# matwilso/generative_models

Measured on AMD Instinct MI355X. Metric: ddpm_train_images_per_sec, higher is better.
Workload: dtype fp16_fwd+bf16_bwd; 1 GPU; DDPM train step, 3x32x32, SimpleUnet C=128, 2048 images per GPU, T=1000 (BASELINE.json configs[2]); key=cfg2, global_batch=2048, parallelism=dp1

## Files before the change

generative_models_amd/csrc/conv1x1_stream.hip:

```cpp
#include <type_traits>

#include "gmk_common.h"

namespace {

constexpr int kRow = 272;

template <typename T>
__global__ __launch_bounds__(256) void conv1x1_pair_stream_kernel(const T* __restrict__ src, const T* __restrict__ w, T* __restrict__ out_a,
                                                                 T* __restrict__ out_b, unsigned npix, unsigned ntiles, unsigned src_bytes) {
    fp16_saturating_stores<T>();
    typedef typename Frag16<T>::type frag_t;
    typedef __attribute__((ext_vector_type(4))) unsigned int u32x4s;
    constexpr unsigned kBadOff = 0xFFFFFF00u;
    __shared__ __attribute__((aligned(16))) char wl[256 * kRow];
    __shared__ __attribute__((aligned(16))) char tile[128 * kRow];
    __shared__ __attribute__((aligned(16))) char trans[4 * 32 * kRow];
    const int tid = threadIdx.x, lane = tid & 63, wave = tid >> 6;
    const int r = lane & 31, h = lane >> 5;
    const __amdgpu_buffer_rsrc_t rss = __builtin_amdgcn_make_buffer_rsrc(const_cast<T*>(src), 0, (int)src_bytes, 0x00020000);
    const __amdgpu_buffer_rsrc_t rsa = __builtin_amdgcn_make_buffer_rsrc(out_a, 0, (int)src_bytes, 0x00020000);
    const __amdgpu_buffer_rsrc_t rsb = __builtin_amdgcn_make_buffer_rsrc(out_b, 0, (int)src_bytes, 0x00020000);
#pragma unroll
    for (int i = 0; i < 16; ++i) {
// ... 145 lines not shown
                s16x4 hi = __builtin_amdgcn_ds_read_tr16_b64_v4i16((GMK_LDS s16x4*)(Yb + (pxl + 4) * 256 + wa));
                const s16x8 t = {lo[0], lo[1], lo[2], lo[3], hi[0], hi[1], hi[2], hi[3]};
                a[i] = __builtin_bit_cast(bf16x8, t);
                lo = __builtin_amdgcn_ds_read_tr16_b64_v4i16((GMK_LDS s16x4*)(Xb + pxl * 256 + wb));
                hi = __builtin_amdgcn_ds_read_tr16_b64_v4i16((GMK_LDS s16x4*)(Xb + (pxl + 4) * 256 + wb));
                const s16x8 u = {lo[0], lo[1], lo[2], lo[3], hi[0], hi[1], hi[2], hi[3]};
                b[i] = __builtin_bit_cast(bf16x8, u);
            }
#pragma unroll
            for (int i = 0; i < 2; ++i)
#pragma unroll
                for (int j = 0; j < 2; ++j) acc[i][j] = __builtin_amdgcn_mfma_f32_32x32x16_bf16(a[i], b[j], acc[i][j], 0, 0, 0);
        }
        if (ks + 1 < nk) write_step(PAR ^ 1, ry[PAR ^ 1], rx0[PAR ^ 1], rx1[PAR ^ 1]);
        __syncthreads();
    };
    for (int ks = 0; ks < nk; ks += 2) {
        k_step(ks, std::integral_constant<int, 0>{});
        if (ks + 1 < nk) k_step(ks + 1, std::integral_constant<int, 1>{});
    }
    float* out = slab + (int64_t)blockIdx.x * (128 * 256) + cib * 128;
#pragma unroll
    for (int i = 0; i < 2; ++i)
#pragma unroll
        for (int j = 0; j < 2; ++j)
#pragma unroll
            for (int e = 0; e < 16; ++e) {
                const int co = wm * 64 + i * 32 + (e & 3) + 8 * (e >> 2) + 4 * h;
                const int ci = wn * 64 + j * 32 + r;
                out[co * 256 + ci] = acc[i][j][e];
            }
}

}

int gmk_conv1x1_pair_stream_try(const void* src, int64_t npix, const void* w_rows256, void* out_a, void* out_b, int dtype, hipStream_t stream) {
    if (!gmk_is16(dtype) || gmk_kernel_choice(3, "GMK_DEV_VARIANT") == 46) return 0;
    const int64_t bytes = npix * 256;
    if (bytes >= 0xFFFFFF00ll) return 0;
    const int64_t ntiles = (npix + 127) / 128;
    const int ncu = gmk_cu_limit();
    if (ntiles < 2 * ncu) return 0;
    const unsigned grid = (unsigned)ncu;
    if (dtype == GMK_BF16)
        conv1x1_pair_stream_kernel<bf16_t><<<grid, 256, 0, stream>>>((const bf16_t*)src, (const bf16_t*)w_rows256, (bf16_t*)out_a, (bf16_t*)out_b,
                                                                    (unsigned)npix, (unsigned)ntiles, (unsigned)bytes);
    else
        conv1x1_pair_stream_kernel<f16_t><<<grid, 256, 0, stream>>>((const f16_t*)src, (const f16_t*)w_rows256, (f16_t*)out_a, (f16_t*)out_b,
                                                                   (unsigned)npix, (unsigned)ntiles, (unsigned)bytes);
    return 1;
}

int gmk_conv1x1_wgrad_stream_try(const void* dy, int dy_cstride, const void* src0, const void* src1, int64_t npix, float* slab, int64_t slab_bytes,
                                 bool x_f16, hipStream_t stream) {
    if (gmk_kernel_choice(3, "GMK_DEV_VARIANT") == 47) return 0;
    const int ncu = gmk_cu_limit();
    if (npix < (int64_t)ncu * 64 * 8 || npix >= (1ll << 31) - 64) return 0;
    if (slab_bytes < (int64_t)ncu * 128 * 256 * 4) return 0;
    int64_t chunk = (npix + ncu - 1) / ncu;
    chunk = (chunk + 63) / 64 * 64;
    const int ns = (int)((npix + chunk - 1) / chunk);
    if (x_f16)
        conv1x1_wgrad_stream_kernel<f16_t><<<ns, 512, 0, stream>>>((const bf16_t*)dy, dy_cstride, (const f16_t*)src0, (const f16_t*)src1, slab, (int)npix, (int)chunk);
    else
        conv1x1_wgrad_stream_kernel<bf16_t><<<ns, 512, 0, stream>>>((const bf16_t*)dy, dy_cstride, (const bf16_t*)src0, (const bf16_t*)src1, slab, (int)npix, (int)chunk);
    return ns;
}
```

generative_models_amd/csrc/conv_igemm.hip:

```cpp
#include <stdlib.h>

#include <type_traits>

#include "gmk_common.h"

namespace {

constexpr int kBM = 128, kBN = 128;

struct GatherParams {
    int hs, ws;
    int ho, wo;
    int ksize, pad;
    int mul, shift, mask, lim_h, lim_w;
    signed char ty[9], tx[9];
    unsigned char tapw[9];
    int ntaps;
    int oscale, ooy, oox, out_w, out_hw;
};

__host__ bool make_gather(int mode, int ksize, int hs, int ws, int ho, int wo, GatherParams* g) {
    g->hs = hs; g->ws = ws; g->ho = ho; g->wo = wo;
    g->ksize = ksize; g->pad = ksize == 3 ? 1 : 0;
    g->mul = 1; g->shift = 0; g->mask = 0; g->lim_h = hs; g->lim_w = ws;
// ... 1053 lines not shown
        dim3 grid((p.M + kBM - 1) / kBM, cout / kBN);
        if (dtype == GMK_BF16) conv_igemm_kernel<bf16_t><<<grid, 256, 0, gmk_stream(stream)>>>(p);
        else if (dtype == GMK_F16) conv_igemm_kernel<f16_t><<<grid, 256, 0, gmk_stream(stream)>>>(p);
        else if (fp32_split()) conv_igemm_kernel<float, true><<<grid, 256, 0, gmk_stream(stream)>>>(p);
        else conv_igemm_kernel<float><<<grid, 256, 0, gmk_stream(stream)>>>(p);
    }
    return gmk_check_launch("gmk_conv_igemm");
}

extern "C" int gmk_conv_igemm(const void* src0, const void* src1, int c0, int c1, int B, int hs, int ws, int ho, int wo,
                              int ksize, int mode, const void* w, int w_rows, int n0, int cout, const float* bias,
                              const float* emb, int emb_stride, const void* residual, void* out, int out_cstride,
                              float* gn_stats, int64_t gn_stats_bytes, const float* gn_scale, const float* gn_shift, int gn_stride,
                              int dtype, void* stream) {
    return conv_igemm_impl(src0, src1, c0, c1, B, hs, ws, ho, wo, ksize, mode, w, w_rows, n0, cout, bias, emb, emb_stride, residual,
                           out, nullptr, out_cstride, gn_stats, gn_stats_bytes, gn_scale, gn_shift, gn_stride, dtype, stream);
}

extern "C" int gmk_conv1x1_pair(const void* src, int c, int B, int H, int W, const void* w, int w_rows, int n0, void* out_a,
                                void* out_b, int dtype, void* stream) {
    GMK_REQUIRE(src && w && out_a && out_b, "gmk_conv1x1_pair: null pointer");
    GMK_REQUIRE(n0 >= 0 && n0 + 256 <= w_rows, "gmk_conv1x1_pair: rows n0 .. n0 + 255 outside the %d packed rows", w_rows);
    if (c == 128 && B > 0 && H > 0 && W > 0) {
        const size_t es = 2;
        if (gmk_conv1x1_pair_stream_try(src, (int64_t)B * H * W, (const char*)w + (size_t)n0 * 128 * es, out_a, out_b, dtype, gmk_stream(stream))) {
            gmk_note_kernel(14);
            return gmk_check_launch("gmk_conv1x1_pair(stream)");
        }
    }
    return conv_igemm_impl(src, nullptr, c, 0, B, H, W, H, W, 1, GMK_CONV_NORMAL, w, w_rows, n0, 128, nullptr, nullptr, 0, nullptr,
                           out_a, out_b, 128, nullptr, 0, nullptr, nullptr, 0, dtype, stream);
}

extern "C" int gmk_conv_gn_fusable(int B, int H, int W, int c0, int c1, int cout) {
    const int force = gmk_kernel_choice(0, "GMK_CONV_KERNEL");
    if (force != 0 && force != 3) return 0;
    return gmk_halo_geometry(B, H, W, c0, c1, cout, cout, cout, 1, 0, 1, nullptr);
}

extern "C" int gmk_conv_wgrad(const void* dy, int dy_cstride, const void* src0, const void* src1, int c0, int c1, int B,
                              int hs, int ws, int ho, int wo, int ksize, int mode, float* dw, int cout, void* workspace,
                              int64_t workspace_bytes, int dtype, int x_dtype, void* stream) {
    GMK_REQUIRE(dy && src0 && dw && workspace, "gmk_conv_wgrad: null pointer");
    GMK_REQUIRE(dtype == GMK_BF16 || dtype == GMK_F32, "gmk_conv_wgrad: bad dtype %d", dtype);
    GMK_REQUIRE(x_dtype == dtype || (dtype == GMK_BF16 && x_dtype == GMK_F16),
                "gmk_conv_wgrad: activations of type %d with gradients of type %d (same type, or fp16 activations with bf16 gradients)", x_dtype, dtype);
    const bool xf16 = x_dtype == GMK_F16;
    GMK_REQUIRE(ksize == 1 || ksize == 3, "gmk_conv_wgrad: ksize %d", ksize);
    GMK_REQUIRE(c0 > 0 && c0 % 128 == 0 && c1 >= 0 && c1 % 128 == 0 && (c1 == 0 || src1),
                "gmk_conv_wgrad: source channels must be multiples of 128 (c0=%d c1=%d)", c0, c1);
    GMK_REQUIRE(cout > 0 && cout % 128 == 0 && dy_cstride >= cout, "gmk_conv_wgrad: bad cout=%d", cout);
    GMK_REQUIRE(B > 0 && (int64_t)B * ho * wo < (1ll << 31) - 256 && (int64_t)B * hs * ws < (1ll << 31),
                "gmk_conv_wgrad: problem too large for 32-bit pixel indices");
    GMK_REQUIRE(mode != GMK_CONV_TRANSPOSED2, "gmk_conv_wgrad: no weight gradient for the transposed gather");
    WgradParams p;
    GMK_REQUIRE(make_gather(mode, ksize, hs, ws, ho, wo, &p.g), "gmk_conv_wgrad: mode %d inconsistent with %dx%d -> %dx%d",
                mode, hs, ws, ho, wo);
    const int taps = ksize * ksize;
    const int wforce = gmk_kernel_choice(1, "GMK_WGRAD_KERNEL");
    const bool s2 = mode == GMK_CONV_STRIDE2 && hs == 2 * ho && ws == 2 * wo;
    if (wforce != 1 && dtype == GMK_BF16 && (mode == GMK_CONV_NORMAL || mode == GMK_CONV_UPSAMPLE2 || s2) && ksize == 3) {
        const int ns2 = gmk_conv_wgrad_slots_try(dy, dy_cstride, src0, src1, c0, c1, B, ho, wo, cout, (float*)workspace,
                                                 workspace_bytes, wforce, mode == GMK_CONV_UPSAMPLE2, xf16, gmk_stream(stream), s2);
        if (ns2 > 0) {
            int rc2 = gmk_check_launch("gmk_conv_wgrad(slots)");
            if (rc2) return rc2;
// ... 35 lines not shown
```

generative_models_amd/csrc/gmk_common.h:

```cpp
#pragma once
#include <hip/hip_runtime.h>
#include <stdint.h>

#include "../../include/gmk.h"

typedef __bf16 bf16_t;
typedef __attribute__((ext_vector_type(8))) __bf16 bf16x8;
typedef __attribute__((ext_vector_type(4))) __bf16 bf16x4;
typedef _Float16 f16_t;
typedef __attribute__((ext_vector_type(8))) _Float16 f16x8;
typedef __attribute__((ext_vector_type(4))) _Float16 f16x4;
typedef __attribute__((ext_vector_type(2))) _Float16 f16x2;
typedef __attribute__((ext_vector_type(2))) __bf16 bf16x2;
typedef __attribute__((ext_vector_type(4))) short s16x4;
typedef __attribute__((ext_vector_type(4))) float f32x4;
typedef __attribute__((ext_vector_type(16))) float f32x16;

#define GMK_LDS __attribute__((address_space(3)))

void gmk_set_error(const char* fmt, ...);
int gmk_check_launch(const char* what);
int gmk_kernel_choice(int which, const char* env);
int gmk_conv1x1_pair_stream_try(const void* src, int64_t npix, const void* w_rows256, void* out_a, void* out_b, int dtype, hipStream_t stream);
int gmk_conv1x1_wgrad_stream_try(const void* dy, int dy_cstride, const void* src0, const void* src1, int64_t npix, float* slab, int64_t slab_bytes,
                                 bool x_f16, hipStream_t stream);
int gmk_conv_subpixel_takes(int B, int H, int W, int cin, int cout, int w_rows, int ntaps, int out_cstride, int dtype);
bool fp32_split(void);
int gmk_cu_limit(void);
void gmk_note_kernel(int id);

#define GMK_REQUIRE(cond, ...)                 \
    do {                                       \
        if (!(cond)) {                         \
            gmk_set_error(__VA_ARGS__);        \
            return GMK_ERR_ARG;                \
        }                                      \
    } while (0)

int gmk_conv3x3_halo_try(const void* src0, const void* src1, int c0, int c1, int B, int H, int W, const void* w, int w_rows,
                         int n0, int cout, const float* bias, const float* emb, int emb_stride, const void* residual,
                         void* out, int out_cstride, int min_tiles, int upsample, float* stats, int64_t stats_bytes,
                         const float* gn_scale, const float* gn_shift, int gn_stride, int dtype, hipStream_t stream);

struct HaloGeometry { int R, TP, slots; int64_t rows_total, M, ntiles, nb0, nb1, nbw, nbo; };
int gmk_halo_geometry(int B, int H, int W, int c0, int c1, int w_rows, int cout, int out_cstride, int min_tiles, int upsample,
                      int fused_gn, HaloGeometry* g);

int gmk_wgrad_slots_nsplit(int cout, int ktot);
int gmk_conv_wgrad_slots_try(const void* dy, int dy_cstride, const void* src0, const void* src1, int c0, int c1, int B, int H,
                             int W, int cout, float* slab, int64_t slab_bytes, int forced, int upsample, bool x_f16,
                             hipStream_t stream, int stride2 = 0);


static inline hipStream_t gmk_stream(void* s) { return reinterpret_cast<hipStream_t>(s); }
static inline int gmk_esize(int dtype) { return dtype == GMK_F32 ? 4 : 2; }
static inline bool gmk_is16(int dtype) { return dtype == GMK_BF16 || dtype == GMK_F16; }

template <typename T> struct Vec8;
// ... 145 lines not shown
```

generative_models_amd/diffusion/simple_unet.py:

```python
import math
import os
from collections import OrderedDict

import torch
from torch import nn

from .. import ops

MAX_TIMESTEPS = 256


def _res_names(prefix, cin, cout, emb):
    out = [
        (f"{prefix}.in_layers.0.weight", (cin,)), (f"{prefix}.in_layers.0.bias", (cin,)),
        (f"{prefix}.in_layers.2.weight", (cout, cin, 3, 3)), (f"{prefix}.in_layers.2.bias", (cout,)),
        (f"{prefix}.emb_layers.1.weight", (cout, emb)), (f"{prefix}.emb_layers.1.bias", (cout,)),
        (f"{prefix}.out_layers.0.weight", (cout,)), (f"{prefix}.out_layers.0.bias", (cout,)),
        (f"{prefix}.out_layers.3.weight", (cout, cout, 3, 3)), (f"{prefix}.out_layers.3.bias", (cout,)),
    ]
    if cin != cout:
        out += [(f"{prefix}.skip_connection.weight", (cout, cin, 1, 1)), (f"{prefix}.skip_connection.bias", (cout,))]
    return out


# ... 538 lines not shown
                ops.set_cu_limit(part[0] - part[1])
        for t in tensors:
            t.record_stream(side)

    def _emb_ready(self):
        pend = getattr(self, "_emb_pending", None)
        if pend is not None:
            self._emb_pending = None
            self._join_side()
            pend.record_stream(torch.cuda.current_stream())

    def _join_side(self):
        if self._side is not None:
            torch.cuda.current_stream().wait_stream(self._side)

    def _res_bwd(self, name, ctx, dout, dout_sum, demb_all, blk, extra_add=None, grads=True, defer_skip=False):
        P, G, C = self._pv, self._gv, self.channels
        srcs, a, stats1, h, a2, (mean2, rstd2) = ctx.pop(name)
        B, H, W, _ = dout.shape
        two = len(srcs) == 2
        if grads:
            ops.colsum(dout_sum, G[f"{name}.out_layers.3.bias"], defer=True)
            self._wgrad(dout, [a2], 3, ops.NORMAL, G[f"{name}.out_layers.3.weight"])
        _, wd2 = self._packs[f"{name}.out_layers.3"]
        da2 = self._conv([dout], wd2, C, 3, ops.NORMAL, (H, W))
        dh, dgp, dbp = ops.gn_silu_bwd(da2, h, P[f"{name}.out_layers.0.weight"], P[f"{name}.out_layers.0.bias"], mean2,
                                       rstd2, dxsum=demb_all[:, blk * C:(blk + 1) * C] if grads else None,
                                       dropout=ctx.pop(name + ".dropout", None), xadd=ctx["emb_all"][:, blk * C:(blk + 1) * C])
        if grads:
            ops.colsum(dgp, G[f"{name}.out_layers.0.weight"], defer=True); ops.colsum(dbp, G[f"{name}.out_layers.0.bias"], defer=True)
            ops.colsum(demb_all[:, blk * C:(blk + 1) * C], G[f"{name}.in_layers.2.bias"], defer=True)
            self._wgrad(dh, a, 3, ops.NORMAL, G[f"{name}.in_layers.2.weight"])
        _, wd1 = self._packs[f"{name}.in_layers.2"]
        if two:
            if grads:
                ops.colsum(dout_sum, G[f"{name}.skip_connection.bias"], defer=True)
                self._wgrad(dout, srcs, 1, ops.NORMAL, G[f"{name}.skip_connection.weight"])
            _, wds = self._packs[f"{name}.skip_connection"]
        outs = []
        gw, gb = G[f"{name}.in_layers.0.weight"], G[f"{name}.in_layers.0.bias"]
        if two and C == 128:
            dskips = ops.conv1x1_pair(dout, wds, 2 * C)
        elif two:
            dskips = tuple(self._conv([dout], wds, 2 * C, 1, ops.NORMAL, (H, W), n0=i * C) for i in range(2))
        else:
            dskips = (dout,)
        for i, s in enumerate(srcs):
            da = self._conv([dh], wd1, len(srcs) * C, 3, ops.NORMAL, (H, W), n0=i * C)
            dskip = dskips[i]
            add2 = extra_add[i] if extra_add is not None else None
            gn = (da, dskip, P[f"{name}.in_layers.0.weight"][i * C:(i + 1) * C], P[f"{name}.in_layers.0.bias"][i * C:(i + 1) * C],
                  stats1[i][0], stats1[i][1])
            if defer_skip and i == 1 and grads and C == 128 and not self._narrow and ops.gn_pair_ok(s, self._g2, self._g1, da.dtype):
                outs.append((_DeferredGN(s, gn, gw[C:2 * C], gb[C:2 * C]), None))
                continue
            ssum = torch.empty((B, C), device=dout.device, dtype=torch.float32) if grads else None
            if isinstance(add2, _DeferredGN):
                assert add2.x is s
                ds, (ugp, ubp), (dgp, dbp) = ops.gn_silu_bwd_pair(s, add2.gn, gn, dxsum=ssum)
                ops.colsum(ugp, add2.gw, defer=True); ops.colsum(ubp, add2.gb, defer=True)
            else:
                ds, dgp, dbp = ops.gn_silu_bwd(da, s, *gn[2:], dadd1=dskip, dadd2=add2, dxsum=ssum)
            if grads:
                ops.colsum(dgp, gw[i * C:(i + 1) * C], defer=True); ops.colsum(dbp, gb[i * C:(i + 1) * C], defer=True)
            outs.append((ds, ssum))
        return outs

    def prepare_forward(self, dev=None):
        if self._packs_stale or self._packed_version != self._version_sum():
            self._repack()
        dev = self.flat_params.device if dev is None else dev
        self._freq_table(MAX_TIMESTEPS, dev)
        self._freq_table(4, dev)

# ... 189 lines not shown
```

generative_models_amd/ops.py:

```python
import math

import os

import torch

from ._lib import check, lib

F32, BF16, F16 = 0, 1, 2
_DT = {torch.float32: F32, torch.bfloat16: BF16, torch.float16: F16}
_HALF = (torch.bfloat16, torch.float16)
NORMAL, STRIDE2, UPSAMPLE2, TRANSPOSED2 = 0, 1, 2, 3

PROFILE = None


KERNEL_NAMES = {1: "conv_igemm_kernel", 2: "conv_igemm_dma_kernel", 3: "conv3x3_halo_kernel", 4: "conv3x3_halo_ws_kernel", 11: "conv_wgrad_kernel",
                12: "conv_wgrad_slots_kernel", 13: "conv_wgrad_slots_ws_kernel", 16: "conv_wgrad_subpixel_ws_kernel", 14: "conv1x1_pair_stream_kernel", 15: "conv1x1_wgrad_stream_kernel",
                5: "conv3x3_halo_ws_kernel[zero-stuffed transposed conv]",
                7: "conv3x3_halo_ws_kernel[+1x1 skip]",
                6: "conv_igemm_dma_kernel[stride-2 dgrad phases]",
                17: "conv_wgrad_slots_ws_kernel[stride-2 planes]",
                8: "conv_subpixel_ws_kernel[upsample]", 9: "conv_subpixel_ws_kernel[transposed]", 10: "conv_subpixel_ws_kernel[upsample dgrad]",
                21: "gn_silu_fwd_reg_kernel", 22: "gn_silu_fwd_kernel", 23: "gn_silu_bwd_hybrid_kernel", 24: "gn_silu_bwd_kernel",
                25: "gn_silu_bwd_pair_kernel", 26: "gn_silu_fwd_pair_kernel"}


def instantiation_key(name, dtype):
    if dtype not in _HALF:
        return None
    t = "f16" if dtype == torch.float16 else "bf16"
    if name == "conv3x3_halo_ws_kernel":
        return f"{name}<{t}>"
    if name == "conv3x3_halo_ws_kernel[+1x1 skip]":
        return f"conv3x3_halo_ws_kernel<{t},+skip>"
    if name == "conv_wgrad_slots_ws_kernel[stride-2 planes]":
        return "conv_wgrad_slots_ws_kernel<stride-2 planes>"
    if name.startswith("conv_subpixel_ws_kernel["):
        return f"conv_subpixel_ws_kernel<{t},{name[len('conv_subpixel_ws_kernel['):-1]}>"
    return None


def _nbytes(*tensors):
    if PROFILE is None:
        return 0.0
    return float(sum(t.numel() * t.element_size() for t in tensors if t is not None))


class _Timed:

    def __init__(self, name, flops, nbytes=0.0, fixed=False, multiplied=None, dtype=None):
# ... 81 lines not shown
    _f32(w, "w")
    cout, cin, k, _ = w.shape
    ref = w_fwd if w_fwd is not None else w_dgrad
    for t in (w_fwd, w_dgrad):
        if t is not None:
            _chk(t, name="pack")
            assert t.numel() == w.numel()
    if w_fwd is not None and w_dgrad is not None and w_fwd.dtype != w_dgrad.dtype:
        pack_conv_weight(w, w_fwd, None)
        pack_conv_weight(w, None, w_dgrad)
        return
    check(lib.gmk_pack_conv_weight(_p(w), _p(w_fwd), _p(w_dgrad), cout, cin, k, _DT[ref.dtype], _s()), "pack_conv_weight")


def pack_conv_weights_multi(arena, packs, table, fwd_f16=None):
    import ctypes
    _f32(arena, "arena"); _chk(packs, name="packs")
    n = len(table[0])
    arrs = [(ctypes.c_int * n)(*[int(v) for v in col]) for col in table]
    flags = (ctypes.c_int * n)(*[int(v) for v in fwd_f16]) if fwd_f16 is not None else None
    check(lib.gmk_pack_conv_weights_multi(_p(arena), _p(packs), n, *arrs, flags, _DT[packs.dtype], _s()), "pack_conv_weights_multi")


GN_STATS = False
GN_FUSE = os.environ.get("GMK_GN_FUSE", "1") != "0"
GN_FUSE_MIN_HW = int(os.environ.get("GMK_GN_FUSE_MIN_HW", "2048"))
SKIP_FOLD = os.environ.get("GMK_SKIP_FOLD", "1") != "0"
SKIP_FOLD_OVER_FUSE = os.environ.get("GMK_SKIP_FOLD_FUSE", "fold") != "fuse"
EMB_SIDE = os.environ.get("GMK_EMB_SIDE", "1") == "1"
FWD_SIDE = os.environ.get("GMK_FWD_SIDE", "0") == "1"
WGRAD_CUS = int(os.environ.get("GMK_WGRAD_CUS", "0"))
WGRAD_STREAM = os.environ.get("GMK_WGRAD_STREAM", "1") != "0"
GN_PAIR = os.environ.get("GMK_GN_PAIR", "1") != "0"


def _xadd_stride(xadd, B, C):
    if xadd is None:
        return 0
    assert xadd.dtype == torch.float32 and xadd.shape == (B, C) and xadd.stride(1) == 1 and xadd.is_cuda
    return xadd.stride(0)


def gn_silu_fwd(x, gamma, beta, groups, eps=1e-5, dropout=None, xadd=None):
    _chk(x, name="x"); _f32(gamma, "gamma"); _f32(beta, "beta")
    B, H, W, C = x.shape
    assert gamma.numel() == C and beta.numel() == C
    y = torch.empty_like(x)
    ncol = groups if groups > 0 else (C - groups - 1) // -groups
    mean = torch.empty((B, ncol), device=x.device, dtype=torch.float32)
    rstd = torch.empty_like(mean)
    mean._gn_groups = groups
    st = getattr(x, "_gn_stats", None)
    part, tp, nt = st if st is not None else (None, 0, 0)
    dp, dseed, doff = dropout if dropout is not None else (0.0, 0, 0)
    xs = _xadd_stride(xadd, B, C)
    with _Timed("gn_silu_fwd", 0.0, _nbytes(x, y)):
        check(lib.gmk_gn_silu_fwd(_p(x), _p(y), _p(gamma), _p(beta), _p(mean), _p(rstd), B, H * W, C, groups, eps, _p(part), tp, nt,
                                  float(dp), int(dseed), int(doff), _p(xadd), xs, _DT[x.dtype], _s()), "gn_silu_fwd")
    return y, mean, rstd


def gn_stats(x, gamma, beta, groups, tab_scale, tab_shift, eps=1e-5, xadd=None):
    _chk(x, name="x"); _f32(gamma, "gamma"); _f32(beta, "beta")
    assert x.dtype in _HALF
    B, H, W, C = x.shape
    for t in (tab_scale, tab_shift):
# ... 274 lines not shown
    _f32(bias, "bias"); _f32(bias_sk, "bias_sk")
    assert bias.numel() == cout and bias_sk.numel() == cout
    out = torch.empty((B, H, W, cout), device=s0.device, dtype=s0.dtype)
    with _Timed("conv_igemm", 2.0 * B * H * W * cout * (9 * c0 + 2 * cs), _nbytes(s0, k0, k1, out), dtype=s0.dtype):
        check(lib.gmk_conv3x3_skipfold(_p(s0), c0, B, H, W, _p(w), cout, 0, cout, _p(bias), _p(k0), _p(k1), cs, _p(wsk), cout, 0,
                                       _p(bias_sk), _p(out), cout, _DT[s0.dtype], _s()), "conv3x3_skipfold")
    return out


def conv1x1_pair(src, w, w_rows, n0=0):
    s0 = _chk(src, name="src")
    B, H, W, c = s0.shape
    _chk(w, s0.dtype, "w")
    assert w.numel() == w_rows * c and n0 + 256 <= w_rows
    oa = torch.empty((B, H, W, 128), device=s0.device, dtype=s0.dtype)
    ob = torch.empty_like(oa)
    with _Timed("conv_igemm", 2.0 * B * H * W * 256 * c, _nbytes(s0, oa, ob)):
        check(lib.gmk_conv1x1_pair(_p(s0), c, B, H, W, _p(w), w_rows, n0, _p(oa), _p(ob), _DT[s0.dtype], _s()), "conv1x1_pair")
    return oa, ob


_WS = {}


def _workspace(nbytes, device, tag="conv"):
    key = (tag, device.index, _s())
    ws = _WS.get(key)
    if ws is None or ws.numel() < nbytes:
        ws = torch.empty(int(nbytes), device=device, dtype=torch.uint8)
        _WS[key] = ws
    return ws


def conv_wgrad(dy, srcs, ksize, mode, dw):
    _chk(dy, name="dy")
    s0 = _chk(srcs[0], name="src0")
    s1 = _chk(srcs[1], s0.dtype, "src1") if len(srcs) > 1 else None
    assert s0.dtype == dy.dtype or (s0.dtype == torch.float16 and dy.dtype == torch.bfloat16), (s0.dtype, dy.dtype)
    B, hs, ws_, c0 = s0.shape
    c1 = s1.shape[3] if s1 is not None else 0
    _, ho, wo, cout = dy.shape
    assert dy.shape[0] == B
    assert dw.dtype == torch.float32 and dw.is_contiguous() and dw.numel() == cout * (c0 + c1) * ksize * ksize
    need = lib.gmk_conv_wgrad_workspace_bytes(B * ho * wo, ksize * ksize, cout, c0 + c1)
    assert need > 0
    wsbuf = _workspace(need, dy.device)
    with _Timed("conv_wgrad", 2.0 * B * ho * wo * cout * (c0 + c1) * ksize * ksize, _nbytes(dy, s0, s1)):
        check(lib.gmk_conv_wgrad(_p(dy), cout, _p(s0), _p(s1), c0, c1, B, hs, ws_, ho, wo, ksize, mode, _p(dw), cout,
                                 _p(wsbuf), wsbuf.numel(), _DT[dy.dtype], _DT[s0.dtype], _s()), "conv_wgrad")
    return dw


def conv_wgrad_subpixel_ok(B, H, W, c, dy_dtype, cout=128):
    return dy_dtype == torch.bfloat16 and bool(lib.gmk_conv_wgrad_subpixel_ok(B, H, W, c, cout))


def conv_wgrad_subpixel(dy, x, dw):
    _chk(dy, torch.bfloat16, "dy")
    _chk(x, name="x")
    assert x.dtype in _HALF
    B, H, W, cin = x.shape
    cout = dy.shape[3]
    assert dy.shape == (B, 2 * H, 2 * W, cout)
    assert dw.dtype == torch.float32 and dw.is_contiguous() and dw.numel() == cout * cin * 9
    need = lib.gmk_conv_wgrad_subpixel_workspace_bytes(B, H, W, cin, cout)
    assert need > 0
# ... 509 lines not shown
```

include/gmk.h:

```cpp
#ifndef GMK_H
#define GMK_H
#include <stdint.h>

#ifdef __cplusplus
extern "C" {
#endif

#define GMK_F32 0
#define GMK_BF16 1
#define GMK_F16 2
#define GMK_ERR_ARG (-1)

#define GMK_CONV_NORMAL 0
#define GMK_CONV_STRIDE2 1
#define GMK_CONV_UPSAMPLE2 2
#define GMK_CONV_TRANSPOSED2 3

int gmk_version(void);
const char* gmk_last_error(void);
int gmk_last_kernel(void);
int gmk_set_kernel_choice(int conv, int wgrad, int gn);
int gmk_set_dev_variant(int v);
int gmk_dev_set_stamp_buffer(void* buf, int64_t bytes);
int gmk_set_cu_limit(int n);
// ... 11 lines not shown
                    int B, int HW, int C, int groups, float eps, const float* stats_part, int tile_pixels, int ntiles,
                    float drop_p, uint64_t drop_seed, uint64_t drop_offset, const float* xadd, int xadd_stride, int dtype,
                    void* stream);
int gmk_gn_silu_bwd(const void* dy, const void* x, const float* gamma, const float* beta, const float* mean,
                    const float* rstd, const void* dadd1, const void* dadd2, void* dx, float* dgamma_part,
                    float* dbeta_part, float* dxsum, int dxsum_stride, int B, int HW, int C, int groups,
                    float drop_p, uint64_t drop_seed, uint64_t drop_offset, const float* xadd, int xadd_stride, int dtype,
                    int x_dtype, void* stream);
int gmk_gn_pair_ok(int HW, int C, int groups_a, int groups_b, int x_dtype, int grad_dtype);
int gmk_gn_pair_fwd_ok(int HW, int C, int groups_a, int groups_b, int dtype);
int gmk_gn_silu_fwd_pair(const void* x, void* y_a, void* y_b, const float* gamma_a, const float* beta_a, const float* gamma_b,
                         const float* beta_b, float* mean_a, float* rstd_a, float* mean_b, float* rstd_b, int B, int HW, int C,
                         int groups_a, int groups_b, float eps, const float* xadd, int xadd_stride, int dtype, void* stream);
int gmk_gn_silu_bwd_pair(const void* x, const void* dy_up, const void* dadd_up, const float* gamma_up, const float* beta_up,
                         const float* mean_up, const float* rstd_up, float* dgamma_part_up, float* dbeta_part_up, int groups_up,
                         const void* dy_dn, const void* dadd_dn, const float* gamma_dn, const float* beta_dn, const float* mean_dn,
                         const float* rstd_dn, float* dgamma_part_dn, float* dbeta_part_dn, int groups_dn, void* dx, float* dxsum,
                         int dxsum_stride, int B, int HW, int C, const float* xadd, int xadd_stride, int x_dtype, void* stream);
int gmk_cast16(const void* src, void* dst, int64_t n, int src_dtype, int dst_dtype, void* stream);
int gmk_chansum(const void* x, float* out, int out_stride, int B, int HW, int C, int dtype, void* stream);
int gmk_colsum(const float* part, int64_t stride, float* out, int R, int C, int accumulate, void* stream);
int gmk_colsum_multi(int n, const float* const* part, const int64_t* stride, float* const* out, const int* R,
                     const int* C, void* stream);
int gmk_sumpool2x2(const void* x, void* y, int B, int H, int W, int C, int dtype, void* stream);

int gmk_conv_igemm(const void* src0, const void* src1, int c0, int c1, int B, int hs, int ws, int ho, int wo,
                   int ksize, int mode, const void* w, int w_rows, int n0, int cout, const float* bias,
                   const float* emb, int emb_stride, const void* residual, void* out, int out_cstride,
                   float* gn_stats, int64_t gn_stats_bytes, const float* gn_scale, const float* gn_shift, int gn_stride,
                   int dtype, void* stream);
int gmk_conv_gn_fusable(int B, int H, int W, int c0, int c1, int cout);
int gmk_conv1x1_pair(const void* src, int c, int B, int H, int W, const void* w, int w_rows, int n0, void* out_a, void* out_b,
                     int dtype, void* stream);
int gmk_conv3x3_skipfold_ok(int B, int H, int W, int c0, int cs, int cout);
int gmk_conv3x3_skipfold(const void* src, int c0, int B, int H, int W, const void* w, int w_rows, int n0, int cout,
                         const float* bias, const void* sk0, const void* sk1, int cs, const void* wsk, int wsk_rows, int nsk0,
                         const float* bias_sk, void* out, int out_cstride, int dtype, void* stream);
#define GMK_SUBPIXEL_UPSAMPLE 0
#define GMK_SUBPIXEL_TRANSPOSED 1
#define GMK_SUBPIXEL_UPSAMPLE_DGRAD 2
int gmk_conv_subpixel_ok(int B, int H, int W, int cin, int cout, int dtype);
int gmk_pack_upsample_weight(const float* w, void* w_sub, void* w_sub_dgrad, int cout, int cin, int dtype, int dgrad_dtype, void* stream);
int gmk_conv_subpixel(const void* src, int B, int H, int W, int cin, const void* w, int w_rows, int n0, int cout, int mode,
                      const float* bias, const void* residual, void* out, int out_cstride, int dtype, void* stream);
int gmk_conv_wgrad_subpixel_ok(int B, int H, int W, int cin, int cout);
int64_t gmk_conv_wgrad_subpixel_workspace_bytes(int B, int H, int W, int cin, int cout);
int gmk_conv_wgrad_subpixel(const void* dy, int dy_cstride, const void* x, int B, int H, int W, int cin, int cout, float* dw,
                            void* workspace, int64_t workspace_bytes, int dtype, int x_dtype, void* stream);
int gmk_gn_stats(const void* x, const float* gamma, const float* beta, float* mean, float* rstd, float* tab_scale,
                 float* tab_shift, int tab_stride, int B, int HW, int C, int groups, float eps, const float* xadd,
                 int xadd_stride, int dtype, void* stream);
int gmk_conv_wgrad(const void* dy, int dy_cstride, const void* src0, const void* src1, int c0, int c1, int B,
                   int hs, int ws, int ho, int wo, int ksize, int mode, float* dw, int cout, void* workspace,
                   int64_t workspace_bytes, int dtype, int x_dtype, void* stream);

int gmk_stem_fwd(const float* x, const float* w, const float* bias, void* y, int B, int cin, int H, int W, int C,
                 int dtype, void* stream);
int gmk_stem_wgrad_blocks(int64_t n_pixels);
int gmk_stem_wgrad(const float* x, const void* dy, float* dw_part, int B, int cin, int H, int W, int C, int dtype,
                   void* stream);
int gmk_head_fwd(const void* a, const float* w, const float* bias, float* out, int B, int cout, int H, int W, int C,
                 int dtype, void* stream);
int gmk_head_dgrad(const float* dout, const float* w, void* da, int B, int cout, int H, int W, int C, int dtype,
                   void* stream);
int gmk_head_wgrad_blocks(int64_t n_pixels);
int gmk_head_wgrad(const float* dout, const void* a, float* dw_part, int B, int cout, int H, int W, int C, int dtype,
// ... 74 lines not shown
```

Before: 46470 images/s.

## Fuse 1x1 skip-connection dgrad and wgrad into one streaming kernel

Adds a persistent kernel that reads the bf16 output gradient and both 16-bit skip sources once per pixel tile. From the shared LDS stage it computes both the weight gradient (into a per-block fp32 slab, reduced afterwards) and the two input-gradient halves. In the UNet backward this replaces the separate wgrad stream kernel and the conv1x1 pair kernel, so dy is loaded once instead of twice and one launch goes away. The cost is a larger LDS footprint and more register pressure per block, which may lower per-kernel efficiency.

```diff
diff --git a/generative_models_amd/csrc/conv1x1_stream.hip b/generative_models_amd/csrc/conv1x1_stream.hip
--- a/generative_models_amd/csrc/conv1x1_stream.hip
+++ b/generative_models_amd/csrc/conv1x1_stream.hip
@@ -201,6 +201,168 @@
             }
 }
 
+__device__ __forceinline__ int dual_off(int row, int ch) { return 256 * row + 16 * (ch ^ (((row & 3) << 2) | ((row >> 2) & 3))); }
+
+template <typename TX>
+__global__ __launch_bounds__(512) void conv1x1_skip_bwd_stream_kernel(const bf16_t* __restrict__ dy, const TX* __restrict__ src0,
+                                                                     const TX* __restrict__ src1, const bf16_t* __restrict__ w,
+                                                                     bf16_t* __restrict__ out_a, bf16_t* __restrict__ out_b,
+                                                                     float* __restrict__ slab, int M, int chunk) {
+    typedef __attribute__((ext_vector_type(4))) unsigned int u32x4s;
+    typedef __attribute__((ext_vector_type(8))) short s16x8;
+    constexpr int kStage = 49152, kTrans = 2 * kStage, kTB = 32768;
+    __shared__ __attribute__((aligned(16))) char smem[2 * kStage + 2 * kTB];
+    const int tid = threadIdx.x, lane = tid & 63, wave = tid >> 6;
+    const int wm = wave >> 2, wq = wave & 3, cib = wq >> 1, wn = wq & 1;
+    const int pix_begin = blockIdx.x * chunk;
+    const int pix_end = min(pix_begin + chunk, M);
+    const int nk = pix_end > pix_begin ? (pix_end - pix_begin + 63) / 64 : 0;
+    const int r = lane & 31, h = lane >> 5;
+    bf16x8 af[8];
+#pragma unroll
+    for (int kk = 0; kk < 8; ++kk) af[kk] = *reinterpret_cast<const bf16x8*>(w + (wave * 32 + r) * 128 + 16 * kk + 8 * h);
+    int lds_w[2], srow[2];
+    const int sc = tid & 15;
+#pragma unroll
+    for (int j = 0; j < 2; ++j) {
+        srow[j] = (tid >> 4) + 32 * j;
+        lds_w[j] = dual_off(srow[j], sc);
+    }
+    u32x4s ry[2][2], rx0[2][2], rx1[2][2];
+    auto load_step = [&](int ks, u32x4s (&y)[2], u32x4s (&x0)[2], u32x4s (&x1)[2]) {
+#pragma unroll
+        for (int j = 0; j < 2; ++j) {
+            const int m = pix_begin + ks * 64 + srow[j];
+            u32x4s vy = {0u, 0u, 0u, 0u}, v0 = vy, v1 = vy;
+            if (m < pix_end) {
+                vy = *reinterpret_cast<const u32x4s*>(dy + (int64_t)m * 128 + sc * 8);
+                v0 = *reinterpret_cast<const u32x4s*>(src0 + (int64_t)m * 128 + sc * 8);
+                v1 = *reinterpret_cast<const u32x4s*>(src1 + (int64_t)m * 128 + sc * 8);
+            }
+            y[j] = vy; x0[j] = v0; x1[j] = v1;
+        }
+    };
+    auto round_x = [&](u32x4s v) {
+        if constexpr (!__is_same(TX, bf16_t)) {
+#pragma unroll
+            for (int d = 0; d < 4; ++d) {
+                float lo, hi;
+                unpack_pair<TX>(v[d], lo, hi);
+                v[d] = pack_pair<bf16_t>(lo, hi);
+            }
+        }
+        return v;
+    };
+    auto write_step = [&](int buf, const u32x4s (&y)[2], const u32x4s (&x0)[2], const u32x4s (&x1)[2]) {
+        char* b = smem + buf * kStage;
+#pragma unroll
+        for (int j = 0; j < 2; ++j) {
+            *reinterpret_cast<u32x4s*>(b + lds_w[j]) = y[j];
+            *reinterpret_cast<u32x4s*>(b + 16384 + lds_w[j]) = round_x(x0[j]);
+            *reinterpret_cast<u32x4s*>(b + 32768 + lds_w[j]) = round_x(x1[j]);
+        }
+    };
+    auto flush = [&](int ks) {
+        const char* tb = smem + kTrans + (ks & 1) * kTB;
+#pragma unroll
+        for (int i = 0; i < 4; ++i) {
+            const int id = tid + 512 * i, trow = id >> 4, ch = id & 15;
+            const u32x4s v = *reinterpret_cast<const u32x4s*>(tb + trow * 256 + ((ch ^ (trow & 15)) << 4));
+            const int m = pix_begin + ks * 64 + (trow & 63);
+            if (m < pix_end) *reinterpret_cast<u32x4s*>((trow >> 6 ? out_b : out_a) + (int64_t)m * 128 + ch * 8) = v;
+        }
+    };
+    f32x16 acc[2][2];
+#pragma unroll
+    for (int i = 0; i < 2; ++i)
+#pragma unroll
+        for (int j = 0; j < 2; ++j)
+#pragma unroll
+            for (int e = 0; e < 16; ++e) acc[i][j][e] = 0.f;
+    const int gg = lane >> 4, i16 = lane & 15, q = i16 >> 2, pp = i16 & 3;
+    const int hh = gg >> 1, cblk = gg & 1;
+    if (nk > 0) {
+        load_step(0, ry[0], rx0[0], rx1[0]);
+        if (nk > 1) load_step(1, ry[1], rx0[1], rx1[1]);
+        write_step(0, ry[0], rx0[0], rx1[0]);
+    }
+    __syncthreads();
+    auto k_step = [&](int ks, auto par) {
+        constexpr int PAR = decltype(par)::value;
+        if (ks + 2 < nk) load_step(ks + 2, ry[PAR], rx0[PAR], rx1[PAR]);
+        if (ks > 0) flush(ks - 1);
+        const char* Yb = smem + PAR * kStage;
+        const char* Xb = Yb + 16384 + cib * 16384;
+#pragma unroll
+        for (int kk = 0; kk < 4; ++kk) {
+            bf16x8 a[2], b[2];
+            const int pxl = kk * 16 + 8 * hh + q;
+#pragma unroll
+            for (int i = 0; i < 2; ++i) {
+                const int cha = (wm * 2 + i) * 4 + 2 * cblk + (pp >> 1), chb = (wn * 2 + i) * 4 + 2 * cblk + (pp >> 1);
+                const int sub = 8 * (pp & 1);
+                s16x4 lo = __builtin_amdgcn_ds_read_tr16_b64_v4i16((GMK_LDS s16x4*)(Yb + dual_off(pxl, cha) + sub));
+                s16x4 hi = __builtin_amdgcn_ds_read_tr16_b64_v4i16((GMK_LDS s16x4*)(Yb + dual_off(pxl + 4, cha) + sub));
+                const s16x8 t = {lo[0], lo[1], lo[2], lo[3], hi[0], hi[1], hi[2], hi[3]};
+                a[i] = __builtin_bit_cast(bf16x8, t);
+                lo = __builtin_amdgcn_ds_read_tr16_b64_v4i16((GMK_LDS s16x4*)(Xb + dual_off(pxl, chb) + sub));
+                hi = __builtin_amdgcn_ds_read_tr16_b64_v4i16((GMK_LDS s16x4*)(Xb + dual_off(pxl + 4, chb) + sub));
+                const s16x8 u = {lo[0], lo[1], lo[2], lo[3], hi[0], hi[1], hi[2], hi[3]};
+                b[i] = __builtin_bit_cast(bf16x8, u);
+            }
+#pragma unroll
+            for (int i = 0; i < 2; ++i)
+#pragma unroll
+                for (int j = 0; j < 2; ++j) acc[i][j] = __builtin_amdgcn_mfma_f32_32x32x16_bf16(a[i], b[j], acc[i][j], 0, 0, 0);
+        }
+        char* tb = smem + kTrans + PAR * kTB;
+#pragma unroll
+        for (int pg = 0; pg < 2; ++pg) {
+            const int p = pg * 32 + r;
+            f32x16 d;
+#pragma unroll
+            for (int e = 0; e < 16; ++e) d[e] = 0.f;
+#pragma unroll
+            for (int kk = 0; kk < 8; ++kk) {
+                const bf16x8 bf = *reinterpret_cast<const bf16x8*>(Yb + dual_off(p, 2 * kk + h));
+                d = __builtin_amdgcn_mfma_f32_32x32x16_bf16(af[kk], bf, d, 0, 0, 0);
+            }
+            unsigned pk[4][2];
+#pragma unroll
+            for (int q4 = 0; q4 < 4; ++q4) {
+                pk[q4][0] = pack_pair<bf16_t>(d[4 * q4], d[4 * q4 + 1]);
+                pk[q4][1] = pack_pair<bf16_t>(d[4 * q4 + 2], d[4 * q4 + 3]);
+            }
+            const int trow = wm * 64 + p;
+#pragma unroll
+            for (int q4 = 0; q4 < 4; q4 += 2) {
+                const auto s0 = __builtin_amdgcn_permlane32_swap(pk[q4][0], pk[q4 + 1][0], false, false);
+                const auto s1 = __builtin_amdgcn_permlane32_swap(pk[q4][1], pk[q4 + 1][1], false, false);
+                const u32x4s o = {s0[0], s1[0], s0[1], s1[1]};
+                *reinterpret_cast<u32x4s*>(tb + trow * 256 + ((((wq * 4 + q4 + h)) ^ (trow & 15)) << 4)) = o;
+            }
+        }
+        if (ks + 1 < nk) write_step(PAR ^ 1, ry[PAR ^ 1], rx0[PAR ^ 1], rx1[PAR ^ 1]);
+        __syncthreads();
+    };
+    for (int ks = 0; ks < nk; ks += 2) {
+        k_step(ks, std::integral_constant<int, 0>{});
+        if (ks + 1 < nk) k_step(ks + 1, std::integral_constant<int, 1>{});
+    }
+    if (nk > 0) flush(nk - 1);
+    float* out = slab + (int64_t)blockIdx.x * (128 * 256) + cib * 128;
+#pragma unroll
+    for (int i = 0; i < 2; ++i)
+#pragma unroll
+        for (int j = 0; j < 2; ++j)
+#pragma unroll
+            for (int e = 0; e < 16; ++e) {
+                const int co = wm * 64 + i * 32 + (e & 3) + 8 * (e >> 2) + 4 * h;
+                const int ci = wn * 64 + j * 32 + r;
+                out[co * 256 + ci] = acc[i][j][e];
+            }
+}
+
 }
 
 int gmk_conv1x1_pair_stream_try(const void* src, int64_t npix, const void* w_rows256, void* out_a, void* out_b, int dtype, hipStream_t stream) {
@@ -235,3 +397,29 @@
         conv1x1_wgrad_stream_kernel<bf16_t><<<ns, 512, 0, stream>>>((const bf16_t*)dy, dy_cstride, (const bf16_t*)src0, (const bf16_t*)src1, slab, (int)npix, (int)chunk);
     return ns;
 }
+
+int gmk_conv1x1_skip_bwd_plan(int64_t npix, int64_t* chunk) {
+    const int dv = gmk_kernel_choice(3, "GMK_DEV_VARIANT");
+    if (dv == 46 || dv == 47) return 0;
+    const int ncu = gmk_cu_limit();
+    if (npix < (int64_t)ncu * 64 * 8 || npix * 256 >= 0xFFFFFF00ll) return 0;
+    if ((npix + 127) / 128 < 2 * ncu) return 0;
+    int64_t ch = (npix + ncu - 1) / ncu;
+    ch = (ch + 63) / 64 * 64;
+    if (chunk) *chunk = ch;
+    return (int)((npix + ch - 1) / ch);
+}
+
+int gmk_conv1x1_skip_bwd_stream_try(const void* dy, const void* src0, const void* src1, int64_t npix, const void* w_rows256, void* out_a, void* out_b,
+                                    float* slab, int64_t slab_bytes, bool x_f16, hipStream_t stream) {
+    int64_t chunk = 0;
+    const int ns = gmk_conv1x1_skip_bwd_plan(npix, &chunk);
+    if (ns <= 0 || slab_bytes < (int64_t)ns * 128 * 256 * 4) return 0;
+    if (x_f16)
+        conv1x1_skip_bwd_stream_kernel<f16_t><<<ns, 512, 0, stream>>>((const bf16_t*)dy, (const f16_t*)src0, (const f16_t*)src1, (const bf16_t*)w_rows256,
+                                                                      (bf16_t*)out_a, (bf16_t*)out_b, slab, (int)npix, (int)chunk);
+    else
+        conv1x1_skip_bwd_stream_kernel<bf16_t><<<ns, 512, 0, stream>>>((const bf16_t*)dy, (const bf16_t*)src0, (const bf16_t*)src1, (const bf16_t*)w_rows256,
+                                                                       (bf16_t*)out_a, (bf16_t*)out_b, slab, (int)npix, (int)chunk);
+    return ns;
+}
diff --git a/generative_models_amd/csrc/conv_igemm.hip b/generative_models_amd/csrc/conv_igemm.hip
--- a/generative_models_amd/csrc/conv_igemm.hip
+++ b/generative_models_amd/csrc/conv_igemm.hip
@@ -1109,6 +1109,33 @@
                            out_a, out_b, 128, nullptr, 0, nullptr, nullptr, 0, dtype, stream);
 }
 
+extern "C" int gmk_conv1x1_skip_bwd_ok(int B, int H, int W, int c, int grad_dtype, int x_dtype) {
+    if (B <= 0 || H <= 0 || W <= 0 || c != 128 || grad_dtype != GMK_BF16 || (x_dtype != GMK_BF16 && x_dtype != GMK_F16)) return 0;
+    if (gmk_kernel_choice(1, "GMK_WGRAD_KERNEL") == 1) return 0;
+    return gmk_conv1x1_skip_bwd_plan((int64_t)B * H * W, nullptr) > 0;
+}
+
+extern "C" int64_t gmk_conv1x1_skip_bwd_workspace_bytes(int B, int H, int W) {
+    const int ns = gmk_conv1x1_skip_bwd_plan((int64_t)B * H * W, nullptr);
+    return ns > 0 ? (int64_t)ns * 128 * 256 * 4 : -1;
+}
+
+extern "C" int gmk_conv1x1_skip_bwd(const void* dy, const void* src0, const void* src1, int B, int H, int W, const void* w, int w_rows, int n0,
+                                    void* out_a, void* out_b, float* dw, void* workspace, int64_t workspace_bytes, int x_dtype, void* stream) {
+    GMK_REQUIRE(dy && src0 && src1 && w && out_a && out_b && dw && workspace, "gmk_conv1x1_skip_bwd: null pointer");
+    GMK_REQUIRE(n0 >= 0 && n0 + 256 <= w_rows, "gmk_conv1x1_skip_bwd: rows n0 .. n0 + 255 outside the %d packed rows", w_rows);
+    GMK_REQUIRE(gmk_conv1x1_skip_bwd_ok(B, H, W, 128, GMK_BF16, x_dtype),
+                "gmk_conv1x1_skip_bwd: unsupported shape B=%d H=%d W=%d x_dtype=%d (gmk_conv1x1_skip_bwd_ok)", B, H, W, x_dtype);
+    const int ns = gmk_conv1x1_skip_bwd_stream_try(dy, src0, src1, (int64_t)B * H * W, (const char*)w + (size_t)n0 * 128 * 2, out_a, out_b,
+                                                   (float*)workspace, workspace_bytes, x_dtype == GMK_F16, gmk_stream(stream));
+    GMK_REQUIRE(ns > 0, "gmk_conv1x1_skip_bwd: workspace of %lld bytes too small (gmk_conv1x1_skip_bwd_workspace_bytes)", (long long)workspace_bytes);
+    gmk_note_kernel(18);
+    int rc = gmk_check_launch("gmk_conv1x1_skip_bwd");
+    if (rc) return rc;
+    launch_wgrad_reduce((const float*)workspace, dw, ns, 1, 128, 256, gmk_stream(stream));
+    return gmk_check_launch("gmk_conv1x1_skip_bwd(reduce)");
+}
+
 extern "C" int gmk_conv_gn_fusable(int B, int H, int W, int c0, int c1, int cout) {
     const int force = gmk_kernel_choice(0, "GMK_CONV_KERNEL");
     if (force != 0 && force != 3) return 0;
diff --git a/generative_models_amd/csrc/gmk_common.h b/generative_models_amd/csrc/gmk_common.h
--- a/generative_models_amd/csrc/gmk_common.h
+++ b/generative_models_amd/csrc/gmk_common.h
@@ -24,6 +24,9 @@
 int gmk_conv1x1_pair_stream_try(const void* src, int64_t npix, const void* w_rows256, void* out_a, void* out_b, int dtype, hipStream_t stream);
 int gmk_conv1x1_wgrad_stream_try(const void* dy, int dy_cstride, const void* src0, const void* src1, int64_t npix, float* slab, int64_t slab_bytes,
                                  bool x_f16, hipStream_t stream);
+int gmk_conv1x1_skip_bwd_plan(int64_t npix, int64_t* chunk);
+int gmk_conv1x1_skip_bwd_stream_try(const void* dy, const void* src0, const void* src1, int64_t npix, const void* w_rows256, void* out_a, void* out_b,
+                                    float* slab, int64_t slab_bytes, bool x_f16, hipStream_t stream);
 int gmk_conv_subpixel_takes(int B, int H, int W, int cin, int cout, int w_rows, int ntaps, int out_cstride, int dtype);
 bool fp32_split(void);
 int gmk_cu_limit(void);
diff --git a/generative_models_amd/diffusion/simple_unet.py b/generative_models_amd/diffusion/simple_unet.py
--- a/generative_models_amd/diffusion/simple_unet.py
+++ b/generative_models_amd/diffusion/simple_unet.py
@@ -594,14 +594,18 @@
             ops.colsum(demb_all[:, blk * C:(blk + 1) * C], G[f"{name}.in_layers.2.bias"], defer=True)
             self._wgrad(dh, a, 3, ops.NORMAL, G[f"{name}.in_layers.2.weight"])
         _, wd1 = self._packs[f"{name}.in_layers.2"]
+        fuse_skip = two and grads and C == 128 and ops.conv1x1_skip_bwd_ok(dout, srcs)
         if two:
             if grads:
                 ops.colsum(dout_sum, G[f"{name}.skip_connection.bias"], defer=True)
-                self._wgrad(dout, srcs, 1, ops.NORMAL, G[f"{name}.skip_connection.weight"])
+                if not fuse_skip:
+                    self._wgrad(dout, srcs, 1, ops.NORMAL, G[f"{name}.skip_connection.weight"])
             _, wds = self._packs[f"{name}.skip_connection"]
         outs = []
         gw, gb = G[f"{name}.in_layers.0.weight"], G[f"{name}.in_layers.0.bias"]
-        if two and C == 128:
+        if fuse_skip:
+            dskips = ops.conv1x1_skip_bwd(dout, srcs, wds, 2 * C, G[f"{name}.skip_connection.weight"])
+        elif two and C == 128:
             dskips = ops.conv1x1_pair(dout, wds, 2 * C)
         elif two:
             dskips = tuple(self._conv([dout], wds, 2 * C, 1, ops.NORMAL, (H, W), n0=i * C) for i in range(2))
diff --git a/generative_models_amd/ops.py b/generative_models_amd/ops.py
--- a/generative_models_amd/ops.py
+++ b/generative_models_amd/ops.py
@@ -16,6 +16,7 @@
 
 KERNEL_NAMES = {1: "conv_igemm_kernel", 2: "conv_igemm_dma_kernel", 3: "conv3x3_halo_kernel", 4: "conv3x3_halo_ws_kernel", 11: "conv_wgrad_kernel",
                 12: "conv_wgrad_slots_kernel", 13: "conv_wgrad_slots_ws_kernel", 16: "conv_wgrad_subpixel_ws_kernel", 14: "conv1x1_pair_stream_kernel", 15: "conv1x1_wgrad_stream_kernel",
+                18: "conv1x1_skip_bwd_stream_kernel",
                 5: "conv3x3_halo_ws_kernel[zero-stuffed transposed conv]",
                 7: "conv3x3_halo_ws_kernel[+1x1 skip]",
                 6: "conv_igemm_dma_kernel[stride-2 dgrad phases]",
@@ -163,6 +164,7 @@
 WGRAD_CUS = int(os.environ.get("GMK_WGRAD_CUS", "0"))
 WGRAD_STREAM = os.environ.get("GMK_WGRAD_STREAM", "1") != "0"
 GN_PAIR = os.environ.get("GMK_GN_PAIR", "1") != "0"
+SKIP_BWD_FUSE = os.environ.get("GMK_SKIP_BWD_FUSE", "1") != "0"
 
 
 def _xadd_stride(xadd, B, C):
@@ -503,6 +505,42 @@
     return ws
 
 
+def _skip_bwd_operands(dy, srcs):
+    if len(srcs) != 2 or dy.dim() != 4 or dy.dtype != torch.bfloat16 or srcs[0].dtype not in _HALF or srcs[1].dtype != srcs[0].dtype:
+        return None
+    if tuple(srcs[0].shape) != tuple(dy.shape) or tuple(srcs[1].shape) != tuple(dy.shape):
+        return None
+    return tuple(dy.shape)
+
+
+def conv1x1_skip_bwd_ok(dy, srcs):
+    dims = _skip_bwd_operands(dy, srcs) if SKIP_BWD_FUSE else None
+    if dims is None:
+        return False
+    B, H, W, c = dims
+    return bool(lib.gmk_conv1x1_skip_bwd_ok(B, H, W, c, _DT[dy.dtype], _DT[srcs[0].dtype]))
+
+
+def conv1x1_skip_bwd(dy, srcs, w, w_rows, dw, n0=0):
+    dims = _skip_bwd_operands(dy, srcs)
+    if dims is None:
+        raise ValueError("conv1x1_skip_bwd: need a bf16 gradient and two 16-bit sources of its shape")
+    B, H, W, c = dims
+    _chk(dy, name="dy"); _chk(srcs[0], name="src0"); _chk(srcs[1], name="src1"); _chk(w, dy.dtype, "w")
+    assert c == 128 and w.numel() == w_rows * c and n0 + 256 <= w_rows
+    assert dw.dtype == torch.float32 and dw.is_contiguous() and dw.is_cuda and dw.numel() == 128 * 256
+    need = lib.gmk_conv1x1_skip_bwd_workspace_bytes(B, H, W)
+    if need <= 0:
+        raise ValueError(f"conv1x1_skip_bwd: shape {dims} is not taken (conv1x1_skip_bwd_ok)")
+    wsbuf = _workspace(need, dy.device)
+    oa = torch.empty((B, H, W, 128), device=dy.device, dtype=dy.dtype)
+    ob = torch.empty_like(oa)
+    with _Timed("conv1x1_skip_bwd_stream_kernel", 2 * 2.0 * B * H * W * 256 * c, _nbytes(dy, srcs[0], srcs[1], oa, ob) + 2.0 * need, fixed=True):
+        check(lib.gmk_conv1x1_skip_bwd(_p(dy), _p(srcs[0]), _p(srcs[1]), B, H, W, _p(w), w_rows, n0, _p(oa), _p(ob), _p(dw), _p(wsbuf),
+                                       wsbuf.numel(), _DT[srcs[0].dtype], _s()), "conv1x1_skip_bwd")
+    return oa, ob
+
+
 def conv_wgrad(dy, srcs, ksize, mode, dw):
     _chk(dy, name="dy")
     s0 = _chk(srcs[0], name="src0")
diff --git a/include/gmk.h b/include/gmk.h
--- a/include/gmk.h
+++ b/include/gmk.h
@@ -67,6 +67,10 @@
 int gmk_conv_gn_fusable(int B, int H, int W, int c0, int c1, int cout);
 int gmk_conv1x1_pair(const void* src, int c, int B, int H, int W, const void* w, int w_rows, int n0, void* out_a, void* out_b,
                      int dtype, void* stream);
+int gmk_conv1x1_skip_bwd_ok(int B, int H, int W, int c, int grad_dtype, int x_dtype);
+int64_t gmk_conv1x1_skip_bwd_workspace_bytes(int B, int H, int W);
+int gmk_conv1x1_skip_bwd(const void* dy, const void* src0, const void* src1, int B, int H, int W, const void* w, int w_rows, int n0,
+                         void* out_a, void* out_b, float* dw, void* workspace, int64_t workspace_bytes, int x_dtype, void* stream);
 int gmk_conv3x3_skipfold_ok(int B, int H, int W, int c0, int cs, int cout);
 int gmk_conv3x3_skipfold(const void* src, int c0, int B, int H, int W, const void* w, int w_rows, int n0, int cout,
                          const float* bias, const void* sk0, const void* sk1, int cs, const void* wsk, int wsk_rows, int nsk0,
```

Result: no change. 46730 images/s, median of 6 (+0.6%).
